# robot-learning-freiburg/MM-DistillNet

Measured on AMD Instinct MI355X. Metric: distillation-step images/sec (3 teachers + audio student, D2, bs=8), higher is better.
Workload: dtype f32; 1 GPU; BASELINE configs[2]: full 3-teacher (RGB+thermal+depth) -> audio student distillation step, EfficientDet-D2, 512x512, per-GPU batch 8, fwd+losses+bwd+all-reduce+Adam; global_batch=8, image_size=512, parallelism=dp1, graph=True, full=False

## Files before the change

include/mmdistill.h:

```cpp
#ifndef MMDISTILL_H
#define MMDISTILL_H
#include <hip/hip_runtime_api.h>
#ifdef __cplusplus
extern "C" {
#endif

#define MMD_ACT_NONE 0
#define MMD_ACT_SWISH 1
#define MMD_ACT_SIGMOID 2

int mmd_bifpn_fuse_fwd(const float* in0, const float* in1, const float* up, const float* pool, const float* theta, float* out, int B, int H, int W, int C, hipStream_t stream);

int mmd_bifpn_node_dw_fwd(const float* in0, const float* in1, const float* up, const float* pool, const float* theta, const float* w_dw, float* f_out, float* zd, int B, int H, int W, int C, hipStream_t stream);

int mmd_bifpn_node_fused_supported(int C);
int mmd_bifpn_node_fwd_fused(const float* in0, const float* in1, const float* up, const float* pool, const float* theta, const float* w_dw, const float* w_pw, const float* bias, const float* scale, const float* shift, float* y, int B, int H, int W, int C, hipStream_t stream);

int mmd_bifpn_node_fwd_fused_train(const float* in0, const float* in1, const float* up, const float* pool, const float* theta, const float* w_dw, const float* w_pw, const float* bias, float* z, float* zd, double* stats, int B, int H, int W, int C, hipStream_t stream);

int mmd_bifpn_fuse_bwd(const float* in0, const float* in1, const float* up, const float* pool, const float* theta, const float* df, float* dx, float* wdot, int B, int H, int W, int C, float* d0, int acc0, float* d1, int acc1, hipStream_t stream);

int mmd_bifpn_node_dw_bwd(const float* in0, const float* in1, const float* up, const float* pool, const float* theta, const float* w_dw, const float* dzd, float* dx, float* wdot, int B, int H, int W, int C, float* d0, int acc0, float* d1, int acc1, float* dup, int acc_up, float* dw_grad, hipStream_t stream);

int mmd_bifpn_node_dw_bwd2(const float* in0, const float* in1, const float* up, const float* pool, const float* theta, const float* w_dw, const float* dzd, float* dx, float* wdot, int B, int H, int W, int C, float* d0, int acc0, float* d1, int acc1, float* dup, int acc_up, float* dw_grad, const float* z0, const float* mean0, const float* invstd0, double* sums0, const float* z1, const float* mean1, const float* invstd1, double* sums1, const float* zu, const float* meanu, const float* invstdu, double* sumsu, hipStream_t stream);
// ... 65 lines not shown

int mmd_stem_im2col(const float* x, float* col, int B, int Cin, int H, int W, int Kp, hipStream_t stream);
int mmd_stem_conv_bwd_weight_supported(int Cin, int H, int W, int Kp, int Cout);
int mmd_stem_wgrad_ws_floats(int Cout);
int mmd_stem_conv_bwd_weight(const float* x, const float* dz, float* dw, float* ws, int B, int Cin, int H, int W, int Kp, int Cout, hipStream_t stream);
int mmd_stem_conv_bwd_weight_bn(const float* x, const float* g, const float* z, float* dw, float* ws, int B, int Cin, int H, int W, int Kp, int Cout, const float* scale, const float* shift, const float* mean, const float* invstd, const double* sums, long long count, int act, float* dgamma, float* dbeta, hipStream_t stream);

int mmd_sigmoid_bwd(const float* dprob, const float* prob, float* dlogit, long long n, hipStream_t stream);

int mmd_slice_rows(const float* src, float* dst, int B, int rows, int N, long long batch_stride, long long offset, hipStream_t stream);
int mmd_slice_rows_pyr(const float* src, float* dst, const int* pyr_desc, int N, long long batch_stride, const long long* offsets, hipStream_t stream);

int mmd_mta_attention(const float* f, float* a, int rows, int C, float p, hipStream_t stream);

int mmd_mta_kl(const float* a_s, const float* a_t0, const float* a_t1, const float* a_t2, int nteachers, int B, int HW, float T, float* loss, float* da_s, float gscale, int accumulate, hipStream_t stream);

int mmd_mta_kl_multi(const float* const* a_s, const float* const* a_t, float* const* da_s, const int* HW, int nlev, int nteachers, int list_mode, int B, float T, float* loss, float gscale, hipStream_t stream);

int mmd_mta_attention_bwd(const float* f, const float* da, float* df, int rows, int C, float p, int accumulate, hipStream_t stream);

int mmd_at_loss_multi(const float* const* a_s, const float* const* a_t, float* const* da_s, const int* HW, int nlev, int nteachers, int B, float* loss, float gscale, float* ws, hipStream_t stream);

int mmd_focal_loss(const float* cls, const float* reg, const float* anchors, const float* boxes, const int* nbox, int maxg, int B, int A, int NC, int* assign_ws, int* npos_ws, double* acc_ws, float* loss_out, float* dcls, float* dreg, float grad_scale, int to_logit, int* any_boxes, hipStream_t stream);

int mmd_adam_step(float* p, const float* g, float* m, float* v, float* state, const float* hyper, const int* active, float grad_scale, long long n, hipStream_t stream);

int mmd_adam_step_gated(float* p, const float* g, float* m, float* v, float* state_main, float* state_head, const float* hyper, const int* head_active, long long b0, long long e0, long long b1, long long e1, long long b2, long long e2, float grad_scale, long long n, hipStream_t stream);

int mmd_opt_step_gated(int mode, float* p, const float* g, float* m, float* v, float* state_main, float* state_head, const float* hyper6, const int* head_active, long long b0, long long e0, long long b1, long long e1, long long b2, long long e2, float grad_scale, long long n, hipStream_t stream);

int mmd_memset_async(void* p, int value, long long bytes, hipStream_t stream);

int mmd_drop_scale(float* out, const float* keep, int n_skip, int batch, unsigned long long seed, unsigned long long* state, hipStream_t stream);

int mmd_ema_update(const float* p0, float* ema0, long long n0, const float* p1, float* ema1, long long n1, const float* p2, float* ema2, long long n2, float* ema_state, float decay, int warmup, hipStream_t stream);

int mmd_clip_grad_norm(float* g, long long n, float max_norm, double* sumsq_ws, hipStream_t stream);

int mmd_decode_filter(const float* cls, const float* reg, const float* anchors, int B, int A, int NC, float conf_threshold, unsigned long long valid_class_mask, float image_size, float* score_ws, unsigned char* clsid_ws, unsigned char* flags_ws, float* over_scores, float* cand, int* n_over, int* n_keep, int* overflow, int cap, hipStream_t stream);

int mmd_nms_teacher(const float* cand, const int* n_keep, const float* over_scores, const int* label_map, float nms_threshold, int inclusive, float image_size, int B, float* out, int* out_cnt, unsigned long long* mask_ws, int* overflow, int cap, float* big_ws, hipStream_t stream);

int mmd_nms_merge(const float* t0, const int* c0, const float* t1, const int* c1, const float* t2, const int* c2, int nteachers, float iou_threshold, int inclusive, int B, float* boxes, int* nbox, int maxg, unsigned long long* mask_ws, int* overflow, int merge01, int cap, float* big_ws, hipStream_t stream);

int mmd_nms_merge_n(const float* const* srcs, const int* const* cnts, int nsrc, float iou_threshold, int inclusive, int B, float* boxes, int* nbox, int maxg, unsigned long long* mask_ws, int* overflow, int merge01, int cap, float* big_ws, hipStream_t stream);

// ... 177 lines not shown
```

mm_distillnet_amd/csrc/loss.hip:

```cpp
#include "common.h"

__global__ __launch_bounds__(256) void mta_attention_kernel(const float* __restrict__ f, float* __restrict__ a, int rows, int C,
                                                            float p) {
  const int wave = (blockIdx.x * 256 + threadIdx.x) >> 6, lane = threadIdx.x & 63;
  if (wave >= rows) return;
  const float* fr = f + (size_t)wave * C;
  float acc = 0.f;
  for (int c = lane * 4; c < C; c += 256) {
    float4 v = mmd_ld4(fr + c);
    if (p == 2.f) acc += v.x * v.x + v.y * v.y + v.z * v.z + v.w * v.w;
    else acc += powf(v.x, p) + powf(v.y, p) + powf(v.z, p) + powf(v.w, p);
  }
  acc = wave_sum(acc);
  if (lane == 0) a[wave] = acc / (float)C;
}
extern "C" int mmd_mta_attention(const float* f, float* a, int rows, int C, float p, hipStream_t stream) {
  if (!f || !a || rows <= 0 || C <= 0 || (C & 3)) return MMD_EINVAL;
  hipLaunchKernelGGL(mta_attention_kernel, dim3(cdiv((long long)rows * 64, 256)), dim3(256), 0, stream, f, a, rows, C, p);
  return mmd_check_launch();
}

__device__ __forceinline__ float block_sum(float v, float* sm, int tid) {
  v = wave_sum(v);
  __syncthreads();
// ... 317 lines not shown
  for (int b = 0; b < m.B; ++b) s += part[(size_t)i * m.B + b];
  loss[i] = s / ((float)m.B * (float)m.HW[i % nlev]);
}
extern "C" int mmd_at_loss_multi(const float* const* a_s, const float* const* a_t, float* const* da_s, const int* HW, int nlev,
                                 int nteachers, int B, float* loss, float gscale, float* ws, hipStream_t stream) {
  if (!a_s || !a_t || !HW || !loss || !ws || nlev < 1 || nlev > MTA_MAX_LEV || nteachers < 1 || nteachers > MTA_MAX_T || B <= 0)
    return MMD_EINVAL;
  AtMulti m{};
  for (int l = 0; l < nlev; ++l) {
    if (!a_s[l] || HW[l] <= 0) return MMD_EINVAL;
    m.a_s[l] = a_s[l]; m.HW[l] = HW[l]; m.da[l] = da_s ? da_s[l] : nullptr;
    for (int t = 0; t < nteachers; ++t) {
      if (!a_t[t * nlev + l]) return MMD_EINVAL;
      m.a_t[t][l] = a_t[t * nlev + l];
    }
  }
  m.nt = nteachers; m.B = B; m.gscale = gscale; m.part = ws;
  hipLaunchKernelGGL(at_loss_multi_kernel, dim3(B, nlev), dim3(256), 0, stream, m);
  hipLaunchKernelGGL(at_loss_sum_kernel, dim3(1), dim3(64), 0, stream, ws, loss, m, nteachers * nlev, nlev);
  return mmd_check_launch();
}

#define FA_LDS_BOXES 1024
__global__ __launch_bounds__(256) void focal_assign_kernel(const float* __restrict__ anchors, const float* __restrict__ boxes,
                                                           const int* __restrict__ nbox, int maxg, int A, int* __restrict__ assign,
                                                           int* npos) {
  __shared__ float4 sbx[FA_LDS_BOXES];
  __shared__ float sar[FA_LDS_BOXES];
  const int b = blockIdx.y;
  const int a = blockIdx.x * 256 + threadIdx.x;
  const int G = min(nbox[b], maxg);
  const float* bx = boxes + (size_t)b * maxg * 5;
  const int GL = min(G, FA_LDS_BOXES);
  for (int g = threadIdx.x; g < GL; g += 256) {
    const float x1 = bx[g * 5], y1 = bx[g * 5 + 1], x2 = bx[g * 5 + 2], y2 = bx[g * 5 + 3];
    sbx[g] = make_float4(x1, y1, x2, y2);
    sar[g] = (x2 - x1) * (y2 - y1);
  }
  __syncthreads();
  int cnt = 0;
  if (a < A && G > 0) {
    float4 an = mmd_ld4(anchors + (size_t)a * 4);
    float aarea = (an.z - an.x) * (an.w - an.y);
    float best = -INFINITY; int bi = 0;
    for (int g = 0; g < G; ++g) {
      float x1, y1, x2, y2, area;
      if (g < GL) { const float4 q = sbx[g]; x1 = q.x; y1 = q.y; x2 = q.z; y2 = q.w; area = sar[g]; }
      else { x1 = bx[g * 5]; y1 = bx[g * 5 + 1]; x2 = bx[g * 5 + 2]; y2 = bx[g * 5 + 3]; area = (x2 - x1) * (y2 - y1); }
      float iw = fmaxf(fminf(an.w, x2) - fmaxf(an.y, x1), 0.f);
      float ih = fmaxf(fminf(an.z, y2) - fmaxf(an.x, y1), 0.f);
      if (g > 0 && !(iw * ih > 0.f)) continue;
      float ua = fmaxf(aarea + area - iw * ih, 1e-8f);
      float iou = iw * ih / ua;
      if (iou > best) { best = iou; bi = g; }
    }
    int v = best >= 0.5f ? bi : (best < 0.4f ? -2 : -1);
    assign[(size_t)b * A + a] = v;
    cnt = v >= 0;
  }
  unsigned long long m = __ballot(cnt);
  if ((threadIdx.x & 63) == 0 && m) atomicAdd(&npos[b], __popcll(m));
}

__global__ __launch_bounds__(256) void focal_loss_kernel(const float* __restrict__ cls, const float* __restrict__ reg,
                                                         const float* __restrict__ anchors, const float* __restrict__ boxes,
                                                         const int* __restrict__ nbox, const int* __restrict__ assign,
                                                         const int* __restrict__ npos, int maxg, int A, int NC, int B,
                                                         double* acc, float* __restrict__ dcls, float* __restrict__ dreg,
                                                         float gscale, int to_logit) {
  __shared__ double sd[8];
  __shared__ short s_as[256], s_lab[256];
  const int b = blockIdx.y, tid = threadIdx.x;
  const int a0 = blockIdx.x * 256;
  const int a = a0 + tid;
  int total = 0;
  for (int i = 0; i < B; ++i) total += min(nbox[i], maxg);
  const int G = min(nbox[b], maxg);
  const float alpha = 0.25f;
  const int np = G > 0 ? npos[b] : 0;
  const float norm = G > 0 ? fmaxf((float)np, 1.f) : 1.f;
  const float gs = gscale / (float)B / norm;
  double lc = 0.0, lr = 0.0;
  {
    int as = -2, lab = -1;
    if (a < A) {
      float* dr = dreg ? dreg + ((size_t)b * A + a) * 4 : nullptr;
      float g4[4] = {0.f, 0.f, 0.f, 0.f};
      if (total != 0) {
        as = G > 0 ? assign[(size_t)b * A + a] : -2;
        if (as >= 0) {
          const float* bx = boxes + ((size_t)b * maxg + as) * 5;
          lab = (int)bx[4];
          float4 an = mmd_ld4(anchors + (size_t)a * 4);
          float aw = an.w - an.y, ah = an.z - an.x;
          float acx = an.y + 0.5f * aw, acy = an.x + 0.5f * ah;
          float gw = bx[2] - bx[0], gh = bx[3] - bx[1];
          float gcx = bx[0] + 0.5f * gw, gcy = bx[1] + 0.5f * gh;
          gw = fmaxf(gw, 1.f); gh = fmaxf(gh, 1.f);
          float t[4] = {(gcy - acy) / ah, (gcx - acx) / aw, __logf(gh / ah), __logf(gw / aw)};
          const float* r = reg + ((size_t)b * A + a) * 4;
          const float gr = gscale / (float)B / (4.f * (float)np);
#pragma unroll
          for (int k = 0; k < 4; ++k) {
            float diff = r[k] - t[k];
            float ad = fabsf(diff);
            float sgn = diff > 0.f ? 1.f : (diff < 0.f ? -1.f : 0.f);
            if (ad <= 1.f / 9.f) { lr += 4.5 * (double)ad * ad; g4[k] = 9.f * ad * sgn * gr; }
            else { lr += (double)ad - 0.5 / 9.0; g4[k] = sgn * gr; }
          }
          lr /= (4.0 * (double)np);
        }
      }
      if (dr) { dr[0] = g4[0]; dr[1] = g4[1]; dr[2] = g4[2]; dr[3] = g4[3]; }
    }
// ... 28 lines not shown
  } else if ((NC & 3) == 0) {
    for (int e = tid * 4; e < run; e += 1024) {
      const int r = e / NC, c = e - r * NC;
      const int as = s_as[r], lab = s_lab[r];
      const float4 r4 = mmd_ld4(cls + base + e);
      float4 g4v;
      ls += term(r4.x, as, c == lab, g4v.x) + term(r4.y, as, c + 1 == lab, g4v.y) + term(r4.z, as, c + 2 == lab, g4v.z) +
            term(r4.w, as, c + 3 == lab, g4v.w);
      if (dcls) mmd_st4(dcls + base + e, g4v);
    }
  } else {
    for (int e = tid; e < run; e += 256) {
      const int r = e / NC, c = e - r * NC;
      float gv;
      ls += term(cls[base + e], s_as[r], c == s_lab[r], gv);
      if (dcls) dcls[base + e] = gv;
    }
  }
  lc = (double)ls / (double)norm;
  lc = wave_sum_d(lc); lr = wave_sum_d(lr);
  const int wave = threadIdx.x >> 6;
  if ((threadIdx.x & 63) == 0) { sd[wave * 2] = lc; sd[wave * 2 + 1] = lr; }
  __syncthreads();
  if (threadIdx.x == 0) {
    atomicAdd(&acc[b * 2], sd[0] + sd[2] + sd[4] + sd[6]);
    atomicAdd(&acc[b * 2 + 1], sd[1] + sd[3] + sd[5] + sd[7]);
  }
}

__global__ void focal_finalize_kernel(const double* acc, const int* nbox, int maxg, int B, float* out, int* any_boxes) {
  if (threadIdx.x != 0) return;
  int total = 0;
  for (int i = 0; i < B; ++i) total += min(nbox[i], maxg);
  double c = 0, r = 0;
  for (int i = 0; i < B; ++i) { c += acc[i * 2]; r += acc[i * 2 + 1]; }
  out[0] = total ? (float)(r / B) : 0.f;
  out[1] = total ? (float)(c / B) : 0.f;
  if (any_boxes && total) *any_boxes = 1;
}

__global__ void focal_zero_kernel(int* npos, double* acc, int B) {
  for (int i = threadIdx.x; i < B; i += blockDim.x) npos[i] = 0;
  for (int i = threadIdx.x; i < 2 * B; i += blockDim.x) acc[i] = 0.0;
}
extern "C" int mmd_focal_loss(const float* cls, const float* reg, const float* anchors, const float* boxes,
                              const int* nbox, int maxg, int B, int A, int NC, int* assign_ws, int* npos_ws,
                              double* acc_ws, float* loss_out, float* dcls, float* dreg, float grad_scale,
                              int to_logit, int* any_boxes, hipStream_t stream) {
  if (!cls || !reg || !anchors || !boxes || !nbox || !assign_ws || !npos_ws || !acc_ws || !loss_out) return MMD_EINVAL;
  if (B <= 0 || A <= 0 || NC <= 0 || maxg <= 0) return MMD_EINVAL;
  hipLaunchKernelGGL(focal_zero_kernel, dim3(1), dim3(256), 0, stream, npos_ws, acc_ws, B);
  dim3 grid(cdiv(A, 256), B);
  hipLaunchKernelGGL(focal_assign_kernel, grid, dim3(256), 0, stream, anchors, boxes, nbox, maxg, A, assign_ws, npos_ws);
  hipLaunchKernelGGL(focal_loss_kernel, grid, dim3(256), 0, stream, cls, reg, anchors, boxes, nbox, assign_ws, npos_ws, maxg,
                     A, NC, B, acc_ws, dcls, dreg, grad_scale, to_logit);
  hipLaunchKernelGGL(focal_finalize_kernel, dim3(1), dim3(64), 0, stream, acc_ws, nbox, maxg, B, loss_out, any_boxes);
  return mmd_check_launch();
}
```

mm_distillnet_amd/csrc/postproc.hip:

```cpp
#include "common.h"
#include <cfloat>

#define PP_CAP 1024

#define PPS_MAXNC 64
__global__ __launch_bounds__(256) void pp_score_kernel(const float* __restrict__ cls, int A, int NC, float thr,
                                                       unsigned long long valid_mask, float* __restrict__ score,
                                                       unsigned char* __restrict__ clsid, unsigned char* __restrict__ flags) {
  extern __shared__ float spp[];
  const int b = blockIdx.y, tid = threadIdx.x;
  const int a0 = blockIdx.x * 256;
  const int na = min(256, A - a0);
  const size_t base = ((size_t)b * A + a0) * NC;
  const int total = na * NC;
  const int ld = NC + 1;
  if (((base | (size_t)NC) & 3) == 0) {
    for (int e = tid * 4; e < total; e += 1024) {
      const float4 v = mmd_ld4(cls + base + e);
      const int r = e / NC, c = e - r * NC;
      float* d = &spp[r * ld + c];
      d[0] = v.x; d[1] = v.y; d[2] = v.z; d[3] = v.w;
    }
  } else {
    for (int e = tid; e < total; e += 256) { const int r = e / NC; spp[r * ld + (e - r * NC)] = cls[base + e]; }
// ... 130 lines not shown
  float xx2 = fminf(ix2, jx2), yy2 = fminf(iy2, jy2);
  float ww = fmaxf(0.f, __fsub_rn(xx2, xx1)), hh = fmaxf(0.f, __fsub_rn(yy2, yy1));
  float inter = __fmul_rn(ww, hh);
  float ovr = __fdiv_rn(inter, __fsub_rn(__fadd_rn(ia, ja), inter));
  return inclusive ? (ovr >= thr) : (ovr > thr);
}

__device__ __forceinline__ void pp_lds_sort(float* skey, int* sidx, int n, int tid) {
  int PS = 64;
  while (PS < n) PS <<= 1;
  for (int k = 2; k <= PS; k <<= 1)
    for (int j = k >> 1; j > 0; j >>= 1) {
      int ixj = tid ^ j;
      if (ixj > tid && ixj < PS) {
        float k0 = skey[tid], k1 = skey[ixj]; int i0 = sidx[tid], i1 = sidx[ixj];
        bool first_before = (k0 > k1) || (k0 == k1 && i0 < i1);
        bool up = ((tid & k) == 0);
        if (up ? !first_before : first_before) { skey[tid] = k1; skey[ixj] = k0; sidx[tid] = i1; sidx[ixj] = i0; }
      }
      __syncthreads();
    }
}

__global__ __launch_bounds__(1024) void pp_nms_kernel(NmsArgs a) {
  __shared__ float skey[PP_CAP];
  __shared__ int sidx[PP_CAP];
  __shared__ float sbox[PP_CAP * 4];
  __shared__ float sarea[PP_CAP];
  __shared__ unsigned long long smask[3584];
  __shared__ int skeep[PP_CAP];
  __shared__ float sred[16];
  __shared__ unsigned long long sdead[16];
  __shared__ int s_n, s_nk;
  const int b = blockIdx.x, tid = threadIdx.x;
  int cnts[4] = {0, 0, 0, 0}, cnts0[4] = {0, 0, 0, 0}, n = 0, n0 = 0;
  for (int s = 0; s < a.nsrc; ++s) { cnts[s] = min(a.cnt[s][b], a.in_cap); n += cnts[s]; }
  if (a.merge01 && b == 1 && n > 0) {
    for (int s = 0; s < a.nsrc; ++s) { cnts0[s] = min(a.cnt[s][0], a.in_cap); n0 += cnts0[s]; }
    n += n0;
  }
  if (n > PP_CAP && (!a.big_ws || n > a.nmax)) { if (tid == 0) *a.overflow = 1; n = PP_CAP; }
  auto row_ptr = [&](int i) -> const float* {
    int s = 0, img = b;
    if (i < n0) {
      while (s < a.nsrc - 1 && i >= cnts0[s]) { i -= cnts0[s]; ++s; }
      img = 0;
// ... 25 lines not shown
      o[0] = r[0]; o[1] = r[1]; o[2] = r[2]; o[3] = r[3]; o[4] = r[5];
    }
  };
  auto stage_box = [&](int t, int oi) {
    const float* r = row_ptr(oi);
    float off = 0.f;
    if (a.mode == 0) off = __fmul_rn(r[5], __fadd_rn(maxc, 1.f));
    float x1 = __fadd_rn(r[0], off), y1 = __fadd_rn(r[1], off), x2 = __fadd_rn(r[2], off), y2 = __fadd_rn(r[3], off);
    sbox[t * 4] = x1; sbox[t * 4 + 1] = y1; sbox[t * 4 + 2] = x2; sbox[t * 4 + 3] = y2;
    sarea[t] = __fmul_rn(__fsub_rn(x2, x1), __fsub_rn(y2, y1));
  };

  if (n <= PP_CAP) {
    float myscore = -INFINITY;
    if (tid < n) myscore = row_ptr(tid)[4];
    skey[tid] = myscore; sidx[tid] = tid;
    __syncthreads();
    pp_lds_sort(skey, sidx, n, tid);
    if (tid < n) stage_box(tid, sidx[tid]);
    __syncthreads();
    const int words = (n + 63) >> 6;
    const bool in_lds = n * words <= 3584;
    unsigned long long* mask = in_lds ? smask : a.mask_ws + (size_t)b * PP_CAP * (PP_CAP / 64);
    for (int e = tid; e < n * words; e += 1024) {
      int i = e / words, w = e % words;
      unsigned long long bits = 0ull;
      float ix1 = sbox[i * 4], iy1 = sbox[i * 4 + 1], ix2 = sbox[i * 4 + 2], iy2 = sbox[i * 4 + 3], ia = sarea[i];
      int j0 = w * 64;
      for (int q = 0; q < 64; ++q) {
        int j = j0 + q;
        if (j <= i || j >= n) continue;
        if (nms_hit(ix1, iy1, ix2, iy2, ia, sbox[j * 4], sbox[j * 4 + 1], sbox[j * 4 + 2], sbox[j * 4 + 3], sarea[j], a.thr, a.inclusive))
          bits |= 1ull << q;
      }
      mask[(size_t)i * words + w] = bits;
    }
    __syncthreads();
    if (!in_lds) __threadfence();
    __syncthreads();
    if (tid < 64) {
      unsigned long long removed = 0ull;
      int nk = 0;
      for (int i = 0; i < n; ++i) {
        unsigned long long rw = __shfl(removed, i >> 6, 64);
        if (!((rw >> (i & 63)) & 1ull)) {
          if (tid == 0) skeep[nk] = i;
          ++nk;
          if (tid < words) removed |= mask[(size_t)i * words + tid];
        }
      }
      if (tid == 0) { s_nk = nk; s_n = n; }
    }
    __syncthreads();
    int nk = s_nk;
    if (nk > a.out_cap) { if (tid == 0) *a.overflow = 1; nk = a.out_cap; }
    if (tid == 0) a.out_cnt[b] = nk;
    for (int k = tid; k < nk; k += 1024) emit(k, sidx[skeep[k]]);
    return;
  }

  float* ws = a.big_ws + (size_t)b * a.big_stride;
  float* gkey = ws;
  int* gidx = reinterpret_cast<int*>(ws + a.P);
  float* kbox = ws + 2 * (size_t)a.P;
  float* karea = kbox + 4 * (size_t)a.nmax;
  int* kidx = reinterpret_cast<int*>(karea + a.nmax);
  int P = 2048; while (P < n) P <<= 1;
  for (int e = tid; e < P; e += 1024) { gkey[e] = e < n ? row_ptr(e)[4] : -INFINITY; gidx[e] = e; }
  __syncthreads();
  for (int k = 2; k <= P; k <<= 1)
    for (int j = k >> 1; j > 0; j >>= 1) {
      for (int e = tid; e < P; e += 1024) {
        int ixj = e ^ j;
// ... 4 lines not shown
          if (up ? !first_before : first_before) { gkey[e] = k1; gkey[ixj] = k0; gidx[e] = i1; gidx[ixj] = i0; }
        }
      }
      __threadfence_block();
      __syncthreads();
    }
  unsigned long long* mask = a.mask_ws + (size_t)b * PP_CAP * (PP_CAP / 64);
  int nkept = 0;
  for (int c0 = 0; c0 < n; c0 += PP_CAP) {
    const int m = min(PP_CAP, n - c0);
    if (tid < m) { const int oi = gidx[c0 + tid]; sidx[tid] = oi; stage_box(tid, oi); }
    __syncthreads();
    bool alive = tid < m;
    if (alive) {
      const float ix1 = sbox[tid * 4], iy1 = sbox[tid * 4 + 1], ix2 = sbox[tid * 4 + 2], iy2 = sbox[tid * 4 + 3], ia = sarea[tid];
      for (int kk = 0; kk < nkept; ++kk) {
        const float4 kb = *reinterpret_cast<const float4*>(kbox + 4 * (size_t)kk);
        if (nms_hit(kb.x, kb.y, kb.z, kb.w, karea[kk], ix1, iy1, ix2, iy2, ia, a.thr, a.inclusive)) { alive = false; break; }
      }
    }
    const unsigned long long live = __ballot(alive);
    if ((tid & 63) == 0) sdead[tid >> 6] = ~live;
    const int words = (m + 63) >> 6;
    for (int e = tid; e < m * words; e += 1024) {
      int i = e / words, w = e % words;
      unsigned long long bits = 0ull;
      float ix1 = sbox[i * 4], iy1 = sbox[i * 4 + 1], ix2 = sbox[i * 4 + 2], iy2 = sbox[i * 4 + 3], ia = sarea[i];
      int j0 = w * 64;
      for (int q = 0; q < 64; ++q) {
        int j = j0 + q;
        if (j <= i || j >= m) continue;
        if (nms_hit(ix1, iy1, ix2, iy2, ia, sbox[j * 4], sbox[j * 4 + 1], sbox[j * 4 + 2], sbox[j * 4 + 3], sarea[j], a.thr, a.inclusive))
          bits |= 1ull << q;
      }
      mask[(size_t)i * words + w] = bits;
    }
    __threadfence_block();
    __syncthreads();
    if (tid < 64) {
      unsigned long long removed = tid < words ? sdead[tid] : 0ull;
      int nk = 0;
      for (int i = 0; i < m; ++i) {
        unsigned long long rw = __shfl(removed, i >> 6, 64);
        if (!((rw >> (i & 63)) & 1ull)) {
          if (tid == 0) skeep[nk] = i;
          ++nk;
          if (tid < words) removed |= mask[(size_t)i * words + tid];
        }
      }
      if (tid == 0) s_nk = nk;
    }
    __syncthreads();
    const int nkc = s_nk;
    for (int k = tid; k < nkc; k += 1024) {
      const int i = skeep[k];
      *reinterpret_cast<float4*>(kbox + 4 * (size_t)(nkept + k)) = make_float4(sbox[i * 4], sbox[i * 4 + 1], sbox[i * 4 + 2], sbox[i * 4 + 3]);
      karea[nkept + k] = sarea[i];
      kidx[nkept + k] = sidx[i];
    }
    nkept += nkc;
    __threadfence_block();
    __syncthreads();
  }
  int nk = nkept;
  if (nk > a.out_cap) { if (tid == 0) *a.overflow = 1; nk = a.out_cap; }
  if (tid == 0) a.out_cnt[b] = nk;
  for (int k = tid; k < nk; k += 1024) emit(k, kidx[k]);
}

static int pp_pow2(int n) { int p = 2048; while (p < n) p <<= 1; return p; }
extern "C" int mmd_nms_ws_floats(int nmax) { return nmax <= PP_CAP ? 0 : (int)((2ll * pp_pow2(nmax) + 6ll * nmax + 3) / 4 * 4); }

// ... 202 lines not shown
```

mm_distillnet_amd/step.py:

```python
from __future__ import annotations

import contextlib
import ctypes
import numbers
import os

from dataclasses import dataclass, field
from typing import Dict, List, Optional

import numpy as np
import torch

from . import _lib
from .arch import NetSpec, make_spec
from .engine import Net, Feat, NONE, SWISH, pack_nets
from .postproc import LABEL_MERGES, decode_nms, nms_workspace, valid_class_mask, wbf_merge
from .store import Arena

call = _lib.call
TEACHER_ORDER = ("rgb", "depth", "thermal")
OPT_MODES = {"Adam": 0, "AdamW": 1, "SGD": 2}
KD_LOSSES = ("MTALoss", "AttentionLoss", "None")


# ... 58 lines not shown
        self.cfg = cfg
        self.device = device
        self.world_size = world_size
        self.pg = process_group
        self.student = Net(student_spec, device, trainable=True, precision=cfg.precision)
        slot = max(s.stem_out * ((s.in_channels * 9 + 3) // 4 * 4) for s in teacher_specs.values())
        self.teachers: Dict[str, Net] = {m: Net(teacher_specs[m], device, trainable=False, precision=cfg.precision, stem_slot=slot)
                                         for m in TEACHER_ORDER if m in teacher_specs}
        tl = list(self.teachers.values())
        self.pack = (len(tl) > 1 and not os.environ.get("MMD_NO_PACK") and str(device).startswith("cuda")
                     and pack_nets(tl))
        ps = self.student.ps
        n = ps.n_params
        self.exp_avg = torch.zeros(n, device=device)
        self.exp_avg_sq = torch.zeros(n, device=device)
        self.adam_main = torch.zeros(4, device=device)
        self.adam_head = torch.zeros(4, device=device)
        if cfg.optimizer not in OPT_MODES:
            raise Exception(f"Unsupported optimizer {cfg.optimizer}")
        self.opt_mode = OPT_MODES[cfg.optimizer]
        self.lr = float(cfg.lr)
        self.hyper = torch.tensor([cfg.lr, cfg.b1, cfg.b2, cfg.eps, cfg.weight_decay, cfg.momentum], device=device)
        self.head_active = torch.zeros(1, dtype=torch.int32, device=device)
        self.ema_flat = self.ema_rmean = self.ema_rvar = self.ema_state = self._ema_scratch = None
        if cfg.ema_decay > 0:
            self.ema_flat, self.ema_rmean, self.ema_rvar = ps.flat.clone(), ps.rmean.clone(), ps.rvar.clone()
            self.ema_state = torch.zeros(2, device=device)
        self.overflow = torch.zeros(1, dtype=torch.int32, device=device)
        self.ws = Arena(device, 256 << 20)
        self.head_ranges = self._head_ranges()
        nc = student_spec.num_classes
        lm = cfg.label_map if cfg.label_map is not None else list(range(nc))
        self.label_map = torch.tensor(lm, dtype=torch.int32, device=device)
        self.valid_mask = valid_class_mask(cfg.valid_prediction_ids)
        self.cap = int(cfg.cand_cap)
        self._eval: Optional[dict] = None
        self._merge_aux = None
        self.graph = None
        self._graphs: Dict[str, tuple] = {}
        self.concurrent_teachers = True
        self.side_streams: List = []
        self.fork_stream = True if torch.cuda.is_available() and str(device).startswith("cuda") else None
        self.static: Dict[str, torch.Tensor] = {}
        self.out: Dict[str, torch.Tensor] = {}
        self.n_skip = sum(1 for b in student_spec.blocks if b.skip)
        self.ar_split: Optional[int] = self._default_split() if world_size > 1 else None
# ... 27 lines not shown
        return min(e.off for key, e in ps.entries.items() if key.startswith(q))

    def _default_split(self) -> int:
        ps = self.student.ps
        k = 1
        for b in self.student.spec.blocks[1:]:
            if self._block_off(b.idx) > 0.02 * ps.n_conv:
                break
            k = b.idx
        return k

    def grad_buckets(self):
        ps = self.student.ps
        if self.ar_split is None:
            return [[], [(0, ps.n_params)]]
        o = self._block_off(self.ar_split)
        assert o % 4 == 0
        return [[(o, ps.n_conv)], [(0, o), (ps.n_conv, ps.n_params)]]

    def load(self, student_state, teacher_states: Dict[str, dict]):
        self.student.load_state(student_state)
        for m, net in self.teachers.items():
            net.load_state(teacher_states[m])
        self.reset_ema()

    def _ema_pairs(self):
        ps = self.student.ps
        return ((ps.flat, self.ema_flat), (ps.rmean, self.ema_rmean), (ps.rvar, self.ema_rvar))

    def reset_ema(self):
        if self.ema_flat is None:
            return
        for live, ema in self._ema_pairs():
            ema.copy_(live)
        self.ema_state.zero_()

    def ema_updates(self) -> int:
        return int(self.ema_state[0].item())

    def _ema_exchange(self):
        if self._ema_scratch is None:
            self._ema_scratch = torch.empty_like(self.ema_flat)
        for live, ema in self._ema_pairs():
            tmp = self._ema_scratch[:live.numel()]
            tmp.copy_(live); live.copy_(ema); ema.copy_(tmp)

# ... 114 lines not shown
        if aug and B >= 2:
            merged = st._alloc(*audio.shape)
            call("mmd_audio_merge01", audio, merged, audio[0].numel(), B)
            audio = merged
        st.mark_block, st.mark_event = int(os.environ.get("MMD_PACK_STAGGER", "-1")), None
        cls_s, reg_s, feats_s = st.forward(audio, train=train, drop_scale=drop_scale if train else None)
        A = cls_s.shape[1]
        self._caps(A)
        nlv = len(feats_s)
        use_kd = cfg.kd_loss != "None"
        if use_kd:
            _, a_s = self._attention(st)
            da_all = self.ws.alloc((st._pyr["total"],))
            call("mmd_memset_async", da_all, 0, da_all.numel() * 4)
            da = [da_all[st._pyr["row0"][l]:st._pyr["row0"][l] + st._pyr["rows"][l]] for l in range(nlv)]
        nt = len(self.teachers) + (1 if (cfg.kd_mode == "list" and batch.get("aug_rgb") is not None) else 0)
        kd = self.ws.alloc((nt if cfg.kd_mode == "pairwise" else 1, nlv))
        call("mmd_memset_async", kd, 0, kd.numel() * 4)
        rows_t, cnt_t, att_t = [], [], []
        main_stream = torch.cuda.current_stream()
        concurrent = self.concurrent_teachers and torch.cuda.is_available()
        if concurrent and not self.side_streams:
            self.side_streams = [torch.cuda.Stream() for _ in self.teachers]
        passes = [(mod, net, ti, None) for ti, (mod, net) in enumerate(self.teachers.items())]
        if cfg.kd_mode == "list" and batch.get("aug_rgb") is not None:
            if "rgb" not in self.teachers:
                raise ValueError("the augmentation pass runs the RGB teacher")
            passes.append(("augmentation", self.teachers["rgb"], list(self.teachers).index("rgb"), batch["aug_rgb"]))
        s2 = [b.idx for b in next(iter(self.teachers.values())).spec.blocks if b.stride == 2]
        stagger = int(os.environ.get("MMD_STAGGER", str(s2[1] if len(s2) > 1 else -1)))
        prev_net = None
        G = len(self.teachers)
        rows_small = B * (S // 128) ** 2
        net_f = next(iter(self.teachers.values()))
        node_whole = bool(net_f.FUSE_NODE and net_f.ps.flat.is_cuda and
                          _lib.LIB.load().mmd_bifpn_node_fused_supported(net_f.spec.fpn_w) == 1 and
                          (net_f.spec.fpn_w <= 160 or G * rows_small <= net_f.NODE_FUSE_WIDE_MAXROWS))
        use_pack = bool(self.pack and G > 1 and not aug and S % 128 == 0 and
                        (rows_small % 128 == 0 or (rows_small % 32 == 0 and node_whole)))
        npk = min(G, max(2, int(os.environ.get("MMD_PACK_SPLIT", G))))
        if use_pack:
            nets = list(self.teachers.values())[:npk]
            net0 = nets[0]
            side = self.side_streams[0] if concurrent else main_stream
            if concurrent:
                side.wait_event(fork_event)
                if st.mark_event is not None:
                    side.wait_event(st.mark_event)
            with torch.cuda.stream(side):
                net0.begin_step()
                cls_p, reg_p, feats_p = net0.forward([batch[m] for m in list(self.teachers)[:npk]], train=False, pack=nets)
                if teacher_labels is None:
                    rows_p, cnt_p = self._pseudo_labels(net0, cls_p, reg_p, npk * B, A, S)
                if use_kd:
                    _, a_lv = self._attention(net0)
            for gi in range(npk):
                if teacher_labels is not None:
                    r, c = teacher_labels[gi]
                else:
                    r, c = rows_p[gi * B:(gi + 1) * B], cnt_p[gi * B:(gi + 1) * B]
                rows_t.append(r); cnt_t.append(c)
                att_t.append([a_lv[l][gi * B * f.H * f.W:(gi + 1) * B * f.H * f.W] for l, f in enumerate(feats_p)] if use_kd else None)
            passes = [p_ for p_ in passes if p_[3] is not None or p_[2] >= npk]
        for pi, (mod, net, si, xin) in enumerate(passes):
            ti = si if xin is None else G
            side = self.side_streams[si] if concurrent else main_stream
            if concurrent and xin is None:
                side.wait_event(fork_event)
                if stagger >= 0 and prev_net is not None and prev_net.mark_event is not None:
                    side.wait_event(prev_net.mark_event)
                net.mark_block, net.mark_event = stagger, None
                prev_net = net
            with torch.cuda.stream(side):
                net.begin_step()
                cls_t, reg_t, feats_t = net.forward(xin if xin is not None else (audio if mod == "audio" else batch[mod]), train=False)
                if aug and B >= 2 and use_kd:
                    for f in feats_t:
                        call("mmd_avg_image01", f.z, f.H * f.W * f.C)
                if teacher_labels is not None:
                    r, c = teacher_labels[ti]
                else:
                    r, c = self._pseudo_labels(net, cls_t, reg_t, B, A, S)
                at = self._attention(net)[1] if use_kd else None
            rows_t.append(r); cnt_t.append(c); att_t.append(at)
        if concurrent:
            for side in self.side_streams:
                main_stream.wait_stream(side)
        if use_kd:
            vp = ctypes.c_void_p
            p_as = (vp * nlv)(*[t.data_ptr() for t in a_s])
            p_at = (vp * (nt * nlv))(*[att_t[ti][l].data_ptr() for ti in range(nt) for l in range(nlv)])
            p_da = (vp * nlv)(*[t.data_ptr() for t in da])
            hw = (ctypes.c_int * nlv)(*[f.H * f.W for f in feats_s])
            if cfg.kd_loss == "AttentionLoss":
                call("mmd_at_loss_multi", p_as, p_at, p_da, hw, nlv, nt, B, kd, float(cfg.w_kd), self.ws.alloc((nt * nlv * B,)))
            else:
                call("mmd_mta_kl_multi", p_as, p_at, p_da, hw, nlv, nt, 0 if cfg.kd_mode == "pairwise" else 1, B, float(cfg.T), kd,
                     float(cfg.w_kd))
        if train:
            d_all, dfe = None, [None] * nlv
            if use_kd:
                d_all = st._alloc(st._pyr["total"], feats_s[0].C)
                call("mmd_mta_attention_bwd", st._fcat, da_all, d_all, st._pyr["total"], feats_s[0].C, self._att_p(), 0)
                dfe = [d_all[st._pyr["row0"][l]:st._pyr["row0"][l] + st._pyr["rows"][l]] for l in range(nlv)]
        boxes, nbox, G = self._merge(rows_t, cnt_t, B, aug)
        nc = st.spec.num_classes
        assign = self.ws.alloc((B * A,), torch.int32); npos = self.ws.alloc((B,), torch.int32)
        acc = self.ws.alloc((2 * B,), torch.float64); main = self.ws.alloc((2,))
        dcls = st._alloc(B, A, nc); dreg = st._alloc(B, A, 4)
        call("mmd_focal_loss", cls_s, reg_s, st.anchors(S), boxes, nbox, G, B, A, nc, assign, npos, acc, main, dcls, dreg,
             float(cfg.w_main), 1, self.head_active if train else self.ws.alloc((1,), torch.int32))
        if train and not _lib.dev_switch("MMD_DEV_NO_BWD"):
            call("mmd_memset_async", st.ps.grad, 0, st.ps.grad.numel() * 4)
            st.backward(dcls, dreg, dfe, stop_before=self.ar_split, dfeat_pyr=d_all)
        self.out = {"reg": main[0:1], "cls": main[1:2], "kd": kd, "boxes": boxes, "nbox": nbox, "label_aux": self._merge_aux,
                    "cls_s": cls_s, "reg_s": reg_s, "feats_s": feats_s, "rows_t": rows_t, "cnt_t": cnt_t}
        return self.out

    def backward_tail(self):
        if self.ar_split is not None:
            self.student.backward_finish(self.ar_split)

    def init_comm(self, rank: int):
        import torch.distributed as dist
        dll = _lib.LIB.load()
        tok = (ctypes.c_char * 128)()
        if rank == 0:
            rc = dll.mmd_comm_unique_id(ctypes.cast(tok, ctypes.c_void_p))
            if rc != 0:
                raise RuntimeError(f"mmd_comm_unique_id failed with status {rc}")
        box = [bytes(tok)]
        if self.world_size > 1:
            dist.broadcast_object_list(box, src=0, group=self.pg)
        h = ctypes.c_void_p()
        buf = ctypes.create_string_buffer(box[0], 128)
        rc = dll.mmd_comm_init(ctypes.cast(ctypes.pointer(h), ctypes.c_void_p), rank, self.world_size, ctypes.cast(buf, ctypes.c_void_p))
# ... 254 lines not shown
```

Before: 613.0 images/sec.

## Overlap KD loss on side stream, fuse focal loss finalize, rework NMS mask build

The KD attention and loss kernels now run on a dedicated side stream that overlaps with pseudo-label merging and the focal loss. The gradient memset is issued early when teachers run concurrently. An opt-in fused focal loss (env MMD_FOCAL_FUSED) drops the zero and finalize launches by using per-block partial sums plus a last-block reduction, and it caches target boxes per anchor. NMS mask building switches to a lane-per-column ballot, and the keep-scan skips directly to surviving boxes. These changes add stream synchronisation complexity, and the atomic counter reset must stay consistent under graph replay.

```diff
diff --git a/include/mmdistill.h b/include/mmdistill.h
--- a/include/mmdistill.h
+++ b/include/mmdistill.h
@@ -111,6 +111,9 @@
 int mmd_at_loss_multi(const float* const* a_s, const float* const* a_t, float* const* da_s, const int* HW, int nlev, int nteachers, int B, float* loss, float gscale, float* ws, hipStream_t stream);
 
 int mmd_focal_loss(const float* cls, const float* reg, const float* anchors, const float* boxes, const int* nbox, int maxg, int B, int A, int NC, int* assign_ws, int* npos_ws, double* acc_ws, float* loss_out, float* dcls, float* dreg, float grad_scale, int to_logit, int* any_boxes, hipStream_t stream);
+
+int mmd_focal_parts(int A);
+int mmd_focal_loss_fused(const float* cls, const float* reg, const float* anchors, const float* boxes, const int* nbox, int maxg, int B, int A, int NC, int* assign_ws, int* npos_part_ws, float* tgt_ws, double* acc_part_ws, unsigned int* counter, float* loss_out, float* dcls, float* dreg, float grad_scale, int to_logit, int* any_boxes, hipStream_t stream);
 
 int mmd_adam_step(float* p, const float* g, float* m, float* v, float* state, const float* hyper, const int* active, float grad_scale, long long n, hipStream_t stream);
 
diff --git a/mm_distillnet_amd/csrc/loss.hip b/mm_distillnet_amd/csrc/loss.hip
--- a/mm_distillnet_amd/csrc/loss.hip
+++ b/mm_distillnet_amd/csrc/loss.hip
@@ -363,11 +363,14 @@
 }
 
 #define FA_LDS_BOXES 1024
+template <bool FUSED>
 __global__ __launch_bounds__(256) void focal_assign_kernel(const float* __restrict__ anchors, const float* __restrict__ boxes,
                                                            const int* __restrict__ nbox, int maxg, int A, int* __restrict__ assign,
-                                                           int* npos) {
+                                                           int* npos, float4* __restrict__ tbox, float* __restrict__ tlab) {
   __shared__ float4 sbx[FA_LDS_BOXES];
   __shared__ float sar[FA_LDS_BOXES];
+  __shared__ float slb[FUSED ? FA_LDS_BOXES : 1];
+  __shared__ int scnt[4];
   const int b = blockIdx.y;
   const int a = blockIdx.x * 256 + threadIdx.x;
   const int G = min(nbox[b], maxg);
@@ -377,6 +380,7 @@
     const float x1 = bx[g * 5], y1 = bx[g * 5 + 1], x2 = bx[g * 5 + 2], y2 = bx[g * 5 + 3];
     sbx[g] = make_float4(x1, y1, x2, y2);
     sar[g] = (x2 - x1) * (y2 - y1);
+    if (FUSED) slb[g] = bx[g * 5 + 4];
   }
   __syncthreads();
   int cnt = 0;
@@ -398,18 +402,33 @@
     int v = best >= 0.5f ? bi : (best < 0.4f ? -2 : -1);
     assign[(size_t)b * A + a] = v;
     cnt = v >= 0;
+    if (FUSED && v >= 0) {
+      tbox[(size_t)b * A + a] = v < GL ? sbx[v] : make_float4(bx[v * 5], bx[v * 5 + 1], bx[v * 5 + 2], bx[v * 5 + 3]);
+      tlab[(size_t)b * A + a] = v < GL ? slb[v] : bx[v * 5 + 4];
+    }
   }
   unsigned long long m = __ballot(cnt);
-  if ((threadIdx.x & 63) == 0 && m) atomicAdd(&npos[b], __popcll(m));
-}
-
+  if (FUSED) {
+    if ((threadIdx.x & 63) == 0) scnt[threadIdx.x >> 6] = __popcll(m);
+    __syncthreads();
+    if (threadIdx.x == 0) npos[(size_t)b * gridDim.x + blockIdx.x] = scnt[0] + scnt[1] + scnt[2] + scnt[3];
+  } else {
+    if ((threadIdx.x & 63) == 0 && m) atomicAdd(&npos[b], __popcll(m));
+  }
+}
+
+template <bool FUSED>
 __global__ __launch_bounds__(256) void focal_loss_kernel(const float* __restrict__ cls, const float* __restrict__ reg,
                                                          const float* __restrict__ anchors, const float* __restrict__ boxes,
                                                          const int* __restrict__ nbox, const int* __restrict__ assign,
                                                          const int* __restrict__ npos, int maxg, int A, int NC, int B,
                                                          double* acc, float* __restrict__ dcls, float* __restrict__ dreg,
-                                                         float gscale, int to_logit) {
+                                                         float gscale, int to_logit, const float4* __restrict__ tbox,
+                                                         const float* __restrict__ tlab, unsigned int* counter, float* loss_out,
+                                                         int* any_boxes) {
   __shared__ double sd[8];
+  __shared__ double sfin[FUSED ? 512 : 1];
+  __shared__ int snp[4], slast;
   __shared__ short s_as[256], s_lab[256];
   const int b = blockIdx.y, tid = threadIdx.x;
   const int a0 = blockIdx.x * 256;
@@ -418,7 +437,17 @@
   for (int i = 0; i < B; ++i) total += min(nbox[i], maxg);
   const int G = min(nbox[b], maxg);
   const float alpha = 0.25f;
-  const int np = G > 0 ? npos[b] : 0;
+  int np = 0;
+  if (FUSED) {
+    int v = 0;
+    if (G > 0) for (int i = tid; i < (int)gridDim.x; i += 256) v += npos[(size_t)b * gridDim.x + i];
+    for (int o = 32; o > 0; o >>= 1) v += __shfl_down(v, o, 64);
+    if ((tid & 63) == 0) snp[tid >> 6] = v;
+    __syncthreads();
+    np = snp[0] + snp[1] + snp[2] + snp[3];
+  } else {
+    np = G > 0 ? npos[b] : 0;
+  }
   const float norm = G > 0 ? fmaxf((float)np, 1.f) : 1.f;
   const float gs = gscale / (float)B / norm;
   double lc = 0.0, lr = 0.0;
@@ -430,7 +459,14 @@
       if (total != 0) {
         as = G > 0 ? assign[(size_t)b * A + a] : -2;
         if (as >= 0) {
-          const float* bx = boxes + ((size_t)b * maxg + as) * 5;
+          float bx[5];
+          if (FUSED) {
+            const float4 q = tbox[(size_t)b * A + a];
+            bx[0] = q.x; bx[1] = q.y; bx[2] = q.z; bx[3] = q.w; bx[4] = tlab[(size_t)b * A + a];
+          } else {
+            const float* bg = boxes + ((size_t)b * maxg + as) * 5;
+            bx[0] = bg[0]; bx[1] = bg[1]; bx[2] = bg[2]; bx[3] = bg[3]; bx[4] = bg[4];
+          }
           lab = (int)bx[4];
           float4 an = mmd_ld4(anchors + (size_t)a * 4);
           float aw = an.w - an.y, ah = an.z - an.x;
@@ -505,9 +541,36 @@
   const int wave = threadIdx.x >> 6;
   if ((threadIdx.x & 63) == 0) { sd[wave * 2] = lc; sd[wave * 2 + 1] = lr; }
   __syncthreads();
-  if (threadIdx.x == 0) {
-    atomicAdd(&acc[b * 2], sd[0] + sd[2] + sd[4] + sd[6]);
-    atomicAdd(&acc[b * 2 + 1], sd[1] + sd[3] + sd[5] + sd[7]);
+  if (!FUSED) {
+    if (threadIdx.x == 0) {
+      atomicAdd(&acc[b * 2], sd[0] + sd[2] + sd[4] + sd[6]);
+      atomicAdd(&acc[b * 2 + 1], sd[1] + sd[3] + sd[5] + sd[7]);
+    }
+    return;
+  }
+  const unsigned int nparts = gridDim.x * gridDim.y;
+  if (tid == 0) {
+    double* o = acc + ((size_t)b * gridDim.x + blockIdx.x) * 2;
+    o[0] = sd[0] + sd[2] + sd[4] + sd[6];
+    o[1] = sd[1] + sd[3] + sd[5] + sd[7];
+    __threadfence();
+    slast = atomicAdd(counter, 1u) == nparts - 1;
+  }
+  __syncthreads();
+  if (!slast) return;
+  __threadfence();
+  const unsigned int per = (nparts + 255) / 256;
+  double c = 0.0, r = 0.0;
+  for (unsigned int i = tid * per; i < min((tid + 1) * per, nparts); ++i) { c += acc[2 * (size_t)i]; r += acc[2 * (size_t)i + 1]; }
+  sfin[tid * 2] = c; sfin[tid * 2 + 1] = r;
+  __syncthreads();
+  if (tid == 0) {
+    c = 0.0; r = 0.0;
+    for (int t = 0; t < 256; ++t) { c += sfin[t * 2]; r += sfin[t * 2 + 1]; }
+    loss_out[0] = total ? (float)(r / B) : 0.f;
+    loss_out[1] = total ? (float)(c / B) : 0.f;
+    if (any_boxes && total) *any_boxes = 1;
+    atomicExch(counter, 0u);
   }
 }
 
@@ -534,9 +597,29 @@
   if (B <= 0 || A <= 0 || NC <= 0 || maxg <= 0) return MMD_EINVAL;
   hipLaunchKernelGGL(focal_zero_kernel, dim3(1), dim3(256), 0, stream, npos_ws, acc_ws, B);
   dim3 grid(cdiv(A, 256), B);
-  hipLaunchKernelGGL(focal_assign_kernel, grid, dim3(256), 0, stream, anchors, boxes, nbox, maxg, A, assign_ws, npos_ws);
-  hipLaunchKernelGGL(focal_loss_kernel, grid, dim3(256), 0, stream, cls, reg, anchors, boxes, nbox, assign_ws, npos_ws, maxg,
-                     A, NC, B, acc_ws, dcls, dreg, grad_scale, to_logit);
+  hipLaunchKernelGGL(focal_assign_kernel<false>, grid, dim3(256), 0, stream, anchors, boxes, nbox, maxg, A, assign_ws, npos_ws,
+                     (float4*)nullptr, (float*)nullptr);
+  hipLaunchKernelGGL(focal_loss_kernel<false>, grid, dim3(256), 0, stream, cls, reg, anchors, boxes, nbox, assign_ws, npos_ws, maxg,
+                     A, NC, B, acc_ws, dcls, dreg, grad_scale, to_logit, (const float4*)nullptr, (const float*)nullptr,
+                     (unsigned int*)nullptr, (float*)nullptr, (int*)nullptr);
   hipLaunchKernelGGL(focal_finalize_kernel, dim3(1), dim3(64), 0, stream, acc_ws, nbox, maxg, B, loss_out, any_boxes);
   return mmd_check_launch();
 }
+
+extern "C" int mmd_focal_parts(int A) { return A > 0 ? cdiv(A, 256) : 0; }
+extern "C" int mmd_focal_loss_fused(const float* cls, const float* reg, const float* anchors, const float* boxes, const int* nbox,
+                                    int maxg, int B, int A, int NC, int* assign_ws, int* npos_part_ws, float* tgt_ws,
+                                    double* acc_part_ws, unsigned int* counter, float* loss_out, float* dcls, float* dreg,
+                                    float grad_scale, int to_logit, int* any_boxes, hipStream_t stream) {
+  if (!cls || !reg || !anchors || !boxes || !nbox || !assign_ws || !npos_part_ws || !tgt_ws || !acc_part_ws || !counter || !loss_out)
+    return MMD_EINVAL;
+  if (B <= 0 || A <= 0 || NC <= 0 || maxg <= 0 || ((size_t)tgt_ws & 15)) return MMD_EINVAL;
+  dim3 grid(cdiv(A, 256), B);
+  float4* tbox = reinterpret_cast<float4*>(tgt_ws);
+  float* tlab = tgt_ws + 4 * (size_t)B * A;
+  hipLaunchKernelGGL(focal_assign_kernel<true>, grid, dim3(256), 0, stream, anchors, boxes, nbox, maxg, A, assign_ws, npos_part_ws,
+                     tbox, tlab);
+  hipLaunchKernelGGL(focal_loss_kernel<true>, grid, dim3(256), 0, stream, cls, reg, anchors, boxes, nbox, assign_ws, npos_part_ws, maxg,
+                     A, NC, B, acc_part_ws, dcls, dreg, grad_scale, to_logit, tbox, tlab, counter, loss_out, any_boxes);
+  return mmd_check_launch();
+}
diff --git a/mm_distillnet_amd/csrc/postproc.hip b/mm_distillnet_amd/csrc/postproc.hip
--- a/mm_distillnet_amd/csrc/postproc.hip
+++ b/mm_distillnet_amd/csrc/postproc.hip
@@ -176,6 +176,45 @@
     }
 }
 
+__device__ __forceinline__ void pp_build_mask(unsigned long long* mask, int words, int m, int tid, const float* sbox, const float* sarea,
+                                              float thr, int inclusive) {
+  const int lane = tid & 63;
+  for (int i = tid >> 6; i < m; i += 16) {
+    const float ix1 = sbox[i * 4], iy1 = sbox[i * 4 + 1], ix2 = sbox[i * 4 + 2], iy2 = sbox[i * 4 + 3], ia = sarea[i];
+    for (int w = i >> 6; w < words; ++w) {
+      const int j = w * 64 + lane;
+      bool hit = false;
+      if (j > i && j < m)
+        hit = nms_hit(ix1, iy1, ix2, iy2, ia, sbox[j * 4], sbox[j * 4 + 1], sbox[j * 4 + 2], sbox[j * 4 + 3], sarea[j], thr, inclusive);
+      const unsigned long long bits = __ballot(hit);
+      if (lane == 0) mask[(size_t)i * words + w] = bits;
+    }
+  }
+}
+
+__device__ __forceinline__ int pp_keep_scan(const unsigned long long* mask, int words, int m, unsigned long long removed, int* skeep, int tid) {
+  auto word_of = [&](int w) -> unsigned long long {
+    const unsigned int lo = (unsigned int)__builtin_amdgcn_readlane((int)(unsigned int)(removed & 0xffffffffull), w);
+    const unsigned int hi = (unsigned int)__builtin_amdgcn_readlane((int)(unsigned int)(removed >> 32), w);
+    return ((unsigned long long)hi << 32) | lo;
+  };
+  int nk = 0;
+  for (int w = 0; w < words; ++w) {
+    const int nw = min(64, m - w * 64);
+    const unsigned long long valid = nw == 64 ? ~0ull : ((1ull << nw) - 1ull);
+    unsigned long long alive = ~word_of(w) & valid;
+    while (alive) {
+      const int q = __ffsll((long long)alive) - 1;
+      const int i = w * 64 + q;
+      if (tid == 0) skeep[nk] = i;
+      ++nk;
+      if (tid >= w && tid < words) removed |= mask[(size_t)i * words + tid];
+      alive = ~word_of(w) & valid & ~((2ull << q) - 1ull);
+    }
+  }
+  return nk;
+}
+
 __global__ __launch_bounds__(1024) void pp_nms_kernel(NmsArgs a) {
   __shared__ float skey[PP_CAP];
   __shared__ int sidx[PP_CAP];
@@ -247,33 +286,11 @@
     const int words = (n + 63) >> 6;
     const bool in_lds = n * words <= 3584;
     unsigned long long* mask = in_lds ? smask : a.mask_ws + (size_t)b * PP_CAP * (PP_CAP / 64);
-    for (int e = tid; e < n * words; e += 1024) {
-      int i = e / words, w = e % words;
-      unsigned long long bits = 0ull;
-      float ix1 = sbox[i * 4], iy1 = sbox[i * 4 + 1], ix2 = sbox[i * 4 + 2], iy2 = sbox[i * 4 + 3], ia = sarea[i];
-      int j0 = w * 64;
-      for (int q = 0; q < 64; ++q) {
-        int j = j0 + q;
-        if (j <= i || j >= n) continue;
-        if (nms_hit(ix1, iy1, ix2, iy2, ia, sbox[j * 4], sbox[j * 4 + 1], sbox[j * 4 + 2], sbox[j * 4 + 3], sarea[j], a.thr, a.inclusive))
-          bits |= 1ull << q;
-      }
-      mask[(size_t)i * words + w] = bits;
-    }
-    __syncthreads();
-    if (!in_lds) __threadfence();
+    pp_build_mask(mask, words, n, tid, sbox, sarea, a.thr, a.inclusive);
+    if (!in_lds) __threadfence_block();
     __syncthreads();
     if (tid < 64) {
-      unsigned long long removed = 0ull;
-      int nk = 0;
-      for (int i = 0; i < n; ++i) {
-        unsigned long long rw = __shfl(removed, i >> 6, 64);
-        if (!((rw >> (i & 63)) & 1ull)) {
-          if (tid == 0) skeep[nk] = i;
-          ++nk;
-          if (tid < words) removed |= mask[(size_t)i * words + tid];
-        }
-      }
+      const int nk = pp_keep_scan(mask, words, n, 0ull, skeep, tid);
       if (tid == 0) { s_nk = nk; s_n = n; }
     }
     __syncthreads();
@@ -324,32 +341,11 @@
     const unsigned long long live = __ballot(alive);
     if ((tid & 63) == 0) sdead[tid >> 6] = ~live;
     const int words = (m + 63) >> 6;
-    for (int e = tid; e < m * words; e += 1024) {
-      int i = e / words, w = e % words;
-      unsigned long long bits = 0ull;
-      float ix1 = sbox[i * 4], iy1 = sbox[i * 4 + 1], ix2 = sbox[i * 4 + 2], iy2 = sbox[i * 4 + 3], ia = sarea[i];
-      int j0 = w * 64;
-      for (int q = 0; q < 64; ++q) {
-        int j = j0 + q;
-        if (j <= i || j >= m) continue;
-        if (nms_hit(ix1, iy1, ix2, iy2, ia, sbox[j * 4], sbox[j * 4 + 1], sbox[j * 4 + 2], sbox[j * 4 + 3], sarea[j], a.thr, a.inclusive))
-          bits |= 1ull << q;
-      }
-      mask[(size_t)i * words + w] = bits;
-    }
+    pp_build_mask(mask, words, m, tid, sbox, sarea, a.thr, a.inclusive);
     __threadfence_block();
     __syncthreads();
     if (tid < 64) {
-      unsigned long long removed = tid < words ? sdead[tid] : 0ull;
-      int nk = 0;
-      for (int i = 0; i < m; ++i) {
-        unsigned long long rw = __shfl(removed, i >> 6, 64);
-        if (!((rw >> (i & 63)) & 1ull)) {
-          if (tid == 0) skeep[nk] = i;
-          ++nk;
-          if (tid < words) removed |= mask[(size_t)i * words + tid];
-        }
-      }
+      const int nk = pp_keep_scan(mask, words, m, tid < words ? sdead[tid] : 0ull, skeep, tid);
       if (tid == 0) s_nk = nk;
     }
     __syncthreads();
diff --git a/mm_distillnet_amd/step.py b/mm_distillnet_amd/step.py
--- a/mm_distillnet_amd/step.py
+++ b/mm_distillnet_amd/step.py
@@ -104,6 +104,10 @@
         self.lr = float(cfg.lr)
         self.hyper = torch.tensor([cfg.lr, cfg.b1, cfg.b2, cfg.eps, cfg.weight_decay, cfg.momentum], device=device)
         self.head_active = torch.zeros(1, dtype=torch.int32, device=device)
+        self.focal_counter = torch.zeros(1, dtype=torch.int32, device=device)
+        self.focal_fused = os.environ.get("MMD_FOCAL_FUSED") == "1"
+        self.kd_stream = None
+        self.kd_side = True
         self.ema_flat = self.ema_rmean = self.ema_rvar = self.ema_state = self._ema_scratch = None
         if cfg.ema_decay > 0:
             self.ema_flat, self.ema_rmean, self.ema_rvar = ps.flat.clone(), ps.rmean.clone(), ps.rvar.clone()
@@ -177,6 +181,7 @@
         self.student.load_state(student_state)
         for m, net in self.teachers.items():
             net.load_state(teacher_states[m])
+        self.focal_counter.zero_()
         self.reset_ema()
 
     def _ema_pairs(self):
@@ -337,6 +342,12 @@
         concurrent = self.concurrent_teachers and torch.cuda.is_available()
         if concurrent and not self.side_streams:
             self.side_streams = [torch.cuda.Stream() for _ in self.teachers]
+        kd_side = bool(concurrent and self.kd_side and use_kd)
+        will_bwd = bool(train and not _lib.dev_switch("MMD_DEV_NO_BWD"))
+        if kd_side and self.kd_stream is None:
+            self.kd_stream = torch.cuda.Stream()
+        if concurrent and will_bwd:
+            call("mmd_memset_async", st.ps.grad, 0, st.ps.grad.numel() * 4)
         passes = [(mod, net, ti, None) for ti, (mod, net) in enumerate(self.teachers.items())]
         if cfg.kd_mode == "list" and batch.get("aug_rgb") is not None:
             if "rgb" not in self.teachers:
@@ -365,9 +376,13 @@
             with torch.cuda.stream(side):
                 net0.begin_step()
                 cls_p, reg_p, feats_p = net0.forward([batch[m] for m in list(self.teachers)[:npk]], train=False, pack=nets)
+                if kd_side:
+                    self.kd_stream.wait_event(side.record_event())
+                    with torch.cuda.stream(self.kd_stream):
+                        _, a_lv = self._attention(net0)
                 if teacher_labels is None:
                     rows_p, cnt_p = self._pseudo_labels(net0, cls_p, reg_p, npk * B, A, S)
-                if use_kd:
+                if use_kd and not kd_side:
                     _, a_lv = self._attention(net0)
             for gi in range(npk):
                 if teacher_labels is not None:
@@ -398,35 +413,48 @@
                     r, c = self._pseudo_labels(net, cls_t, reg_t, B, A, S)
                 at = self._attention(net)[1] if use_kd else None
             rows_t.append(r); cnt_t.append(c); att_t.append(at)
+        if kd_side:
+            self.kd_stream.wait_event(main_stream.record_event())
+            for side in self.side_streams:
+                self.kd_stream.wait_stream(side)
         if concurrent:
             for side in self.side_streams:
                 main_stream.wait_stream(side)
-        if use_kd:
-            vp = ctypes.c_void_p
-            p_as = (vp * nlv)(*[t.data_ptr() for t in a_s])
-            p_at = (vp * (nt * nlv))(*[att_t[ti][l].data_ptr() for ti in range(nt) for l in range(nlv)])
-            p_da = (vp * nlv)(*[t.data_ptr() for t in da])
-            hw = (ctypes.c_int * nlv)(*[f.H * f.W for f in feats_s])
-            if cfg.kd_loss == "AttentionLoss":
-                call("mmd_at_loss_multi", p_as, p_at, p_da, hw, nlv, nt, B, kd, float(cfg.w_kd), self.ws.alloc((nt * nlv * B,)))
-            else:
-                call("mmd_mta_kl_multi", p_as, p_at, p_da, hw, nlv, nt, 0 if cfg.kd_mode == "pairwise" else 1, B, float(cfg.T), kd,
-                     float(cfg.w_kd))
-        if train:
-            d_all, dfe = None, [None] * nlv
+        d_all, dfe = None, [None] * nlv
+        with torch.cuda.stream(self.kd_stream if kd_side else main_stream):
             if use_kd:
-                d_all = st._alloc(st._pyr["total"], feats_s[0].C)
-                call("mmd_mta_attention_bwd", st._fcat, da_all, d_all, st._pyr["total"], feats_s[0].C, self._att_p(), 0)
-                dfe = [d_all[st._pyr["row0"][l]:st._pyr["row0"][l] + st._pyr["rows"][l]] for l in range(nlv)]
+                vp = ctypes.c_void_p
+                p_as = (vp * nlv)(*[t.data_ptr() for t in a_s])
+                p_at = (vp * (nt * nlv))(*[att_t[ti][l].data_ptr() for ti in range(nt) for l in range(nlv)])
+                p_da = (vp * nlv)(*[t.data_ptr() for t in da])
+                hw = (ctypes.c_int * nlv)(*[f.H * f.W for f in feats_s])
+                if cfg.kd_loss == "AttentionLoss":
+                    call("mmd_at_loss_multi", p_as, p_at, p_da, hw, nlv, nt, B, kd, float(cfg.w_kd), self.ws.alloc((nt * nlv * B,)))
+                else:
+                    call("mmd_mta_kl_multi", p_as, p_at, p_da, hw, nlv, nt, 0 if cfg.kd_mode == "pairwise" else 1, B, float(cfg.T), kd,
+                         float(cfg.w_kd))
+                if train:
+                    d_all = st._alloc(st._pyr["total"], feats_s[0].C)
+                    call("mmd_mta_attention_bwd", st._fcat, da_all, d_all, st._pyr["total"], feats_s[0].C, self._att_p(), 0)
+                    dfe = [d_all[st._pyr["row0"][l]:st._pyr["row0"][l] + st._pyr["rows"][l]] for l in range(nlv)]
         boxes, nbox, G = self._merge(rows_t, cnt_t, B, aug)
         nc = st.spec.num_classes
-        assign = self.ws.alloc((B * A,), torch.int32); npos = self.ws.alloc((B,), torch.int32)
-        acc = self.ws.alloc((2 * B,), torch.float64); main = self.ws.alloc((2,))
+        parts = _lib.LIB.load().mmd_focal_parts(A) if self.focal_fused else 1
+        assign = self.ws.alloc((B * A,), torch.int32); npos = self.ws.alloc((B * parts,), torch.int32)
+        acc = self.ws.alloc((2 * B * parts,), torch.float64); main = self.ws.alloc((2,))
         dcls = st._alloc(B, A, nc); dreg = st._alloc(B, A, 4)
-        call("mmd_focal_loss", cls_s, reg_s, st.anchors(S), boxes, nbox, G, B, A, nc, assign, npos, acc, main, dcls, dreg,
-             float(cfg.w_main), 1, self.head_active if train else self.ws.alloc((1,), torch.int32))
-        if train and not _lib.dev_switch("MMD_DEV_NO_BWD"):
-            call("mmd_memset_async", st.ps.grad, 0, st.ps.grad.numel() * 4)
+        any_boxes = self.head_active if train else self.ws.alloc((1,), torch.int32)
+        if self.focal_fused:
+            call("mmd_focal_loss_fused", cls_s, reg_s, st.anchors(S), boxes, nbox, G, B, A, nc, assign, npos, self.ws.alloc((5 * B * A,)), acc,
+                 self.focal_counter, main, dcls, dreg, float(cfg.w_main), 1, any_boxes)
+        else:
+            call("mmd_focal_loss", cls_s, reg_s, st.anchors(S), boxes, nbox, G, B, A, nc, assign, npos, acc, main, dcls, dreg,
+                 float(cfg.w_main), 1, any_boxes)
+        if kd_side:
+            main_stream.wait_stream(self.kd_stream)
+        if will_bwd:
+            if not concurrent:
+                call("mmd_memset_async", st.ps.grad, 0, st.ps.grad.numel() * 4)
             st.backward(dcls, dreg, dfe, stop_before=self.ar_split, dfeat_pyr=d_all)
         self.out = {"reg": main[0:1], "cls": main[1:2], "kd": kd, "boxes": boxes, "nbox": nbox, "label_aux": self._merge_aux,
                     "cls_s": cls_s, "reg_s": reg_s, "feats_s": feats_s, "rows_t": rows_t, "cnt_t": cnt_t}
```

Measured after the change: 615.5 images/sec (median of 6 runs). Within noise of the previous version (+0.4%).
